# orting/image-feature-extraction

Hardware: AMD Instinct MI355X
Metric: Mvoxels/sec Hessian+eig, 512^3 fp32 3-scale (higher is better)
Workload: dtype f32 storage / f64 line recurrences

## Files before the change

### image-feature-extraction_amd/csrc/ife_capi.hip

```cpp
#include "../../include/ife_hip.h"

#include <hip/hip_runtime.h>

#include <algorithm>
#include <cmath>
#include <cstdarg>
#include <cstdio>
#include <cstdlib>
#include <cstring>
#include <map>
#include <new>
#include <string>
#include <tuple>
#include <type_traits>
#include <vector>

#include "feature_kernels.hpp"
#include "iir_types.hpp"
#include "stats_kernels.hpp"
#include "distance_kernels.hpp"
#include "dense_kernels.hpp"
#define IFE_IIR_NS iir_exact
#define IFE_IIR_FMA 0
#include "iir_kernels.inc"
// ... 359 lines not shown
DerivCoef deriv_coeffs(const ife_volume_desc *v, int dscale_mode) {
  DerivCoef d;
  const double sp[3] = {v->sx, v->sy, v->sz};
  for (int a = 0; a < 3; ++a) {
    const double s1 = 1.0 / sp[a];
    const double s2 = dscale_mode == 1 ? s1 * s1 : s1;
    d.m1[a] = -0.5 * s1;
    d.p1[a] = 0.5 * s1;
    d.a2[a] = 1.0 * s2;
    d.b2[a] = -2.0 * s2;
    d.c2[a] = 1.0 * s2;
  }
  return d;
}

IirGeom geom_for_axis(const ife_volume_desc *v, int axis) {
  IirGeom g;
  g.in_w = 0; g.in_group = 0; g.in_nz = 0;
  const int64_t nx = v->nx, ny = v->ny, nz = v->nz;
  if (axis == 2) {
    g.n = nz; g.nlines = nx * ny; g.sstride = nx * ny; g.inner = nx * ny; g.outer = 0;
  } else if (axis == 1) {
    g.n = ny; g.nlines = nx * nz; g.sstride = nx; g.inner = nx; g.outer = nx * ny;
  } else {
    g.n = nx; g.nlines = ny * nz; g.sstride = 1; g.inner = 1; g.outer = nx;
  }
  return g;
}

size_t ck_pairs(int64_t n, int K) { return (size_t)((n + K - 1) / K); }

int ensure_ck(ife_ctx *ctx, const ife_volume_desc *v, int njobs) {
  const int K = 8;
  size_t need_y = 0;
  for (int a = 0; a < 3; ++a) {
    IirGeom g = geom_for_axis(v, a);
    const size_t np = ck_pairs(g.n, K);
    need_y = std::max(need_y, np * 4 * (size_t)g.nlines * sizeof(double));
  }
  for (int j = 0; j < njobs; ++j) {
    int rc = ensure(ctx, ctx->ck_y[j], need_y);
    if (rc) return rc;
  }
  return IFE_OK;
}

int ensure_slots(ife_ctx *ctx, const ife_volume_desc *v, int nslots) {
  const size_t nb = (size_t)(v->nx * v->ny * v->nz) * sizeof(float);
  for (int s = 0; s < nslots; ++s)
    for (int i = 0; i < 4; ++i) {
      int rc = ensure(ctx, ctx->fld[s][i], nb);
      if (rc) return rc;
    }
  return IFE_OK;
}

struct ZSweepSrc {
  const void *img, *msk;
  int img_dtype, msk_dtype;
  float *tc, *cf;
  int nf;
  bool write_src;
};
int launch_iir(ife_ctx *ctx, const ife_volume_desc *v, int axis, int njobs,
               const float *const *in, float *const *out, const double *sigma,
               int in_y_chunks = 1, const int *order = nullptr ,
               const float *const *in2 = nullptr, const ZSweepSrc *zs = nullptr) {
  if (njobs < 1 || njobs > IIR_MAX_JOBS) return fail(ctx, IFE_E_ARG, "bad job count %d", njobs);
  IirGeom g = geom_for_axis(v, axis);
  if (in_y_chunks > 1) {
    if (axis != 0) return fail(ctx, IFE_E_ARG, "Y-chunked input is only read by the x pass");
    if (v->ny % in_y_chunks || (v->ny / in_y_chunks) % 64)
      return fail(ctx, IFE_E_SIZE, "Y-chunked input needs ny/chunks to be a multiple of 64");
    g.in_w = in_y_chunks;
    g.in_group = v->ny / in_y_chunks;
    g.in_nz = v->nz;
  }
  if ((int64_t)2 * 16 * g.sstride * 4 >= (int64_t)1 << 31 ||
      g.outer * 4 >= (int64_t)1 << 32 || g.nlines * 8 * 3 >= (int64_t)1 << 32)
    return fail(ctx, IFE_E_SIZE, "volume too large for the 32-bit offsets of the line kernels");
  if (in2 && (axis == 0 || 2 * njobs > IIR_MAX_JOBS || ctx->iir_ckpt != 2))
    return fail(ctx, IFE_E_ARG, "the paired form runs on the strided axes with at most %d jobs", IIR_MAX_JOBS / 2);
  if (zs && (axis != 2 || in2 || order || ctx->iir_ckpt != 2 || zs->nf < 1 || zs->nf > 2 || njobs % zs->nf ||
             njobs / zs->nf > IFE_MAX_SLOTS || !zs->img || !zs->tc || (zs->nf == 2 && (!zs->msk || !zs->cf))))
    return fail(ctx, IFE_E_ARG, "the shared sweep runs the Z pass of up to %d scales with pair checkpoints", IFE_MAX_SLOTS);
  int rc = ensure_ck(ctx, v, in2 ? 2 * njobs : njobs);
  if (rc) return rc;
  if (zs && (rc = ensure(ctx, ctx->zs_rec, (size_t)zs->nf * (size_t)g.nlines * sizeof(uint32_t)))) return rc;
  uint32_t any_const = 0;
  const double sp = axis == 0 ? v->sx : axis == 1 ? v->sy : v->sz;
  IirJobs jobs;
  memset(&jobs, 0, sizeof jobs);
  for (int j = 0; j < njobs; ++j) {
    if (!in[j] || !out[j] || in[j] == out[j]) return fail(ctx, IFE_E_ARG, "bad job buffers");
    if ((reinterpret_cast<uintptr_t>(in[j]) | reinterpret_cast<uintptr_t>(out[j])) % 4)
      return fail(ctx, IFE_E_ARG, "field pointers must be aligned to 4 bytes");
    jobs.j[j].in = in[j];
    jobs.j[j].out = out[j];
    jobs.j[j].ck_y = (double *)ctx->ck_y[j].p;
    if (in2) {
      if (!in2[j] || in2[j] == out[j] || reinterpret_cast<uintptr_t>(in2[j]) % 4)
        return fail(ctx, IFE_E_ARG, "bad denominator buffer");
      jobs.j[j].in2 = in2[j];
      jobs.j[j].ck_y2 = (double *)ctx->ck_y[njobs + j].p;
    }
    if (gauss_coeffs_order(sigma[j], sp, order ? order[j] : 0, &jobs.j[j].c))
      return fail(ctx, IFE_E_ARG, "spacing is suspiciously small");
    jobs.j[j].const_lines = 0;
    if (ctx->const_lines && !ctx->iir_fma && (!order || order[j] == 0)) {
      const int64_t len = axis == 0 ? v->nx : axis == 1 ? v->ny : v->nz;
      const std::tuple<double, double, int64_t> key(sigma[j], sp, len);
      auto it = ctx->const_flags.find(key);
      if (it == ctx->const_flags.end()) {
        if (ctx->const_flags.size() > 256) ctx->const_flags.clear();
        it = ctx->const_flags.emplace(key, const_line_flags(jobs.j[j].c, len)).first;
      }
      jobs.j[j].const_lines = it->second;
    }
    any_const |= jobs.j[j].const_lines;
    if (zs) jobs.j[j].line_rec = (const uint32_t *)ctx->zs_rec.p + (size_t)(j % zs->nf) * (size_t)g.nlines;
  }
  g.njobs = njobs;
  g.ngroups = (int32_t)((g.nlines + (in2 ? 127 : 255)) / (in2 ? 128 : 256));
  const dim3 grid((unsigned)((g.ngroups + 7) / 8 * 8 * njobs), 1, 1);
  const int sblock = ctx->iir_block ? ctx->iir_block : 12;
  if (zs) {
    ProfScope pz(ctx, KK_PREP);
    ZSweepArgs za;
    za.img = zs->img; za.msk = zs->msk; za.tc = zs->tc; za.cf = zs->cf;
    za.rec = (uint32_t *)ctx->zs_rec.p;
    za.nf = zs->nf; za.write_src = zs->write_src ? 1 : 0; za.track = any_const ? 1 : 0;
    IirGeom gs = g;
    gs.njobs = zs->nf;
    const dim3 sgrid((unsigned)((gs.ngroups + 7) / 8 * 8 * zs->nf), 1, 1);
    with_iir_kernels(ctx->iir_fma, [&](auto ks) {
      using KS = decltype(ks);
      with_const<8, 10, 12, 16>(sblock, [&](auto K) {
        with_const<1, 2, 3>(njobs / zs->nf, [&](auto S) {
          auto launch = [&](auto ti, auto tm) {
            hipLaunchKernelGGL((KS::template sweep_z<decltype(K)::value, decltype(S)::value, decltype(ti), decltype(tm)>),
                               sgrid, dim3(256), 0, ctx->stream, jobs, gs, za);
          };
          auto with_mask = [&](auto ti) {
            if (zs->msk && zs->msk_dtype == IFE_U16) launch(ti, uint16_t{});
            else launch(ti, uint8_t{});
          };
          if (zs->img_dtype == IFE_F32) with_mask(float{});
          else with_mask(int16_t{});
        });
      });
    });
    IFE_HIP(ctx, hipGetLastError());
  }
  ProfScope ps(ctx, axis == 2 ? KK_IIR_Z : axis == 1 ? KK_IIR_Y : KK_IIR_X);
  with_iir_kernels(ctx->iir_fma, [&](auto ks) {
    using KS = decltype(ks);
    auto launch = [&](auto kernel) { hipLaunchKernelGGL(kernel, grid, dim3(256), 0, ctx->stream, jobs, g); };
    if (zs)
      with_const<8, 10, 12, 16>(sblock, [&](auto K) { launch(KS::template strided<decltype(K)::value, false, true>); });
    else if (in2)
      with_const<8, 10, 12, 16>(sblock, [&](auto K) { launch(KS::template strided<decltype(K)::value, true, false>); });
    else if (axis == 0)
      with_const<8, 16>(ctx->iir_block, [&](auto K) { launch(KS::template contig<decltype(K)::value>); });
    else if (ctx->iir_ckpt == 1)
      with_const<8, 16>(ctx->iir_block, [&](auto K) { launch(KS::template strided1<decltype(K)::value>); });
    else
      with_const<8, 10, 12, 16>(sblock, [&](auto K) { launch(KS::template strided<decltype(K)::value, false, false>); });
// ... 1006 lines not shown
```

### image-feature-extraction_amd/csrc/iir_kernels.inc

```
#include <hip/hip_runtime.h>
#include <stdint.h>

#include <hip/hip_runtime.h>
#include <stdint.h>

#include <stddef.h>

#include <type_traits>

#include "iir_types.hpp"

#if IFE_IIR_FMA
#define IFE_MADD(a, b, acc) fma((a), (b), (acc))
#else
#define IFE_MADD(a, b, acc) ((a) * (b) + (acc))
#endif

namespace ife {
namespace IFE_IIR_NS {




struct IirCoefMain {
// ... 29 lines not shown
  double y1, y2, y3, y4;
};

template <typename C>
__device__ __forceinline__ double causal_step(CausalState &s, double xin, const C &c) {
  const double a = IFE_MADD(s.x3, c.N3, IFE_MADD(s.x2, c.N2, IFE_MADD(s.x1, c.N1, xin * c.N0)));
  const double t = IFE_MADD(s.y4, c.D4, IFE_MADD(s.y3, c.D3, IFE_MADD(s.y2, c.D2, s.y1 * c.D1)));
  const double y = a - t;
  s.x3 = s.x2; s.x2 = s.x1; s.x1 = xin;
  s.y4 = s.y3; s.y3 = s.y2; s.y2 = s.y1; s.y1 = y;
  return y;
}
__device__ __forceinline__ double causal_step_edge(CausalState &s, double xin, const IirCoef &c,
                                                   int64_t i) {
  const double d1 = i < 1 ? c.BN1 : c.D1;
  const double d2 = i < 2 ? c.BN2 : c.D2;
  const double d3 = i < 3 ? c.BN3 : c.D3;
  const double d4 = i < 4 ? c.BN4 : c.D4;
  const double a = IFE_MADD(s.x3, c.N3, IFE_MADD(s.x2, c.N2, IFE_MADD(s.x1, c.N1, xin * c.N0)));
  const double t = IFE_MADD(s.y4, d4, IFE_MADD(s.y3, d3, IFE_MADD(s.y2, d2, s.y1 * d1)));
  const double y = a - t;
  s.x3 = s.x2; s.x2 = s.x1; s.x1 = xin;
  s.y4 = s.y3; s.y3 = s.y2; s.y2 = s.y1; s.y1 = y;
  return y;
}
template <typename C>
__device__ __forceinline__ double anti_step(AntiState &s, double xin, const C &c) {
  const double a = IFE_MADD(s.x4, c.M4, IFE_MADD(s.x3, c.M3, IFE_MADD(s.x2, c.M2, s.x1 * c.M1)));
  const double t = IFE_MADD(s.y4, c.D4, IFE_MADD(s.y3, c.D3, IFE_MADD(s.y2, c.D2, s.y1 * c.D1)));
  const double y = a - t;
  s.x4 = s.x3; s.x3 = s.x2; s.x2 = s.x1; s.x1 = xin;
  s.y4 = s.y3; s.y3 = s.y2; s.y2 = s.y1; s.y1 = y;
  return y;
}
__device__ __forceinline__ double anti_step_edge(AntiState &s, double xin, const IirCoef &c,
                                                 int64_t i, int64_t n) {
  const double d1 = i + 1 >= n ? c.BM1 : c.D1;
  const double d2 = i + 2 >= n ? c.BM2 : c.D2;
  const double d3 = i + 3 >= n ? c.BM3 : c.D3;
  const double d4 = i + 4 >= n ? c.BM4 : c.D4;
  const double a = IFE_MADD(s.x4, c.M4, IFE_MADD(s.x3, c.M3, IFE_MADD(s.x2, c.M2, s.x1 * c.M1)));
  const double t = IFE_MADD(s.y4, d4, IFE_MADD(s.y3, d3, IFE_MADD(s.y2, d2, s.y1 * d1)));
  const double y = a - t;
  s.x4 = s.x3; s.x3 = s.x2; s.x2 = s.x1; s.x1 = xin;
  s.y4 = s.y3; s.y3 = s.y2; s.y2 = s.y1; s.y1 = y;
  return y;
}

using rsrc_t = __amdgpu_buffer_rsrc_t;

__device__ __forceinline__ int64_t uniform64(int64_t v) {
  const uint32_t lo = __builtin_amdgcn_readfirstlane((uint32_t)(uint64_t)v);
  const uint32_t hi = __builtin_amdgcn_readfirstlane((uint32_t)((uint64_t)v >> 32));
  return (int64_t)(((uint64_t)hi << 32) | lo);
}
__device__ __forceinline__ rsrc_t make_rsrc(const void *ubase) {
  return __builtin_amdgcn_make_buffer_rsrc(const_cast<void *>(ubase), 0, -1, 0x00020000);
}
__device__ __forceinline__ rsrc_t make_rsrc_null(const void *ubase) {
  return __builtin_amdgcn_make_buffer_rsrc(const_cast<void *>(ubase), 0, 0, 0x00020000);
}
__device__ __forceinline__ rsrc_t make_rsrc_range(const void *ubase, uint32_t range) {
  return __builtin_amdgcn_make_buffer_rsrc(const_cast<void *>(ubase), 0, (int)range, 0x00020000);
}
__device__ __forceinline__ uint32_t mask_lt(int a, int b) {
  uint32_t m;
  asm("s_sub_i32 %0, %1, %2\n\ts_ashr_i32 %0, %0, 31" : "=s"(m) : "s"(a), "s"(b) : "scc");
  return m;
}
#if defined(IFE_DIAG_NO_OUT)
#define IFE_OUT_RSRC make_rsrc_null
#define IFE_OUT_RSRC_RANGE(ptr, range) make_rsrc_null(ptr)
#else
#define IFE_OUT_RSRC make_rsrc
#define IFE_OUT_RSRC_RANGE(ptr, range) make_rsrc_range((ptr), (range))
#endif
#if defined(IFE_DIAG_NO_CK)
#define IFE_CK_RSRC make_rsrc_null
#else
#define IFE_CK_RSRC make_rsrc
#endif
#if defined(IFE_DIAG_NO_IN)
#define IFE_IN_RSRC make_rsrc_null
#else
#define IFE_IN_RSRC make_rsrc
#endif
__device__ __forceinline__ float buf_ld_f32(rsrc_t r, uint32_t voff, uint32_t soff) {
  return __builtin_bit_cast(float, __builtin_amdgcn_raw_buffer_load_b32(r, voff, soff, 0));
}
#ifndef IFE_IN2_AUX
#define IFE_IN2_AUX 0
#endif
__device__ __forceinline__ float buf_ld_last_f32(rsrc_t r, uint32_t voff, uint32_t soff) {
  return __builtin_bit_cast(float, __builtin_amdgcn_raw_buffer_load_b32(r, voff, soff, IFE_IN2_AUX));
}
__device__ __forceinline__ void buf_st_f32(rsrc_t r, uint32_t voff, uint32_t soff, float v) {
  __builtin_amdgcn_raw_buffer_store_b32(__builtin_bit_cast(uint32_t, v), r, voff, soff, 0);
}
#ifndef IFE_OUT_AUX
#define IFE_OUT_AUX 2
#endif
__device__ __forceinline__ void buf_st_out_f32(rsrc_t r, uint32_t voff, uint32_t soff, float v) {
  __builtin_amdgcn_raw_buffer_store_b32(__builtin_bit_cast(uint32_t, v), r, voff, soff, IFE_OUT_AUX);
}
typedef uint32_t u32x2 __attribute__((ext_vector_type(2)));
typedef uint32_t u32x4 __attribute__((ext_vector_type(4)));
#ifndef IFE_CK_ST_AUX
#define IFE_CK_ST_AUX 0
#endif
#ifndef IFE_CK_LD_AUX
#define IFE_CK_LD_AUX 0
#endif
__device__ __forceinline__ double ck_ld_f64(rsrc_t r, uint32_t voff, uint32_t soff) {
  return __builtin_bit_cast(double, __builtin_amdgcn_raw_buffer_load_b64(r, voff, soff, IFE_CK_LD_AUX));
}
__device__ __forceinline__ void ck_st_f64(rsrc_t r, uint32_t voff, uint32_t soff, double v) {
  __builtin_amdgcn_raw_buffer_store_b64(__builtin_bit_cast(u32x2, v), r, voff, soff, IFE_CK_ST_AUX);
}
__device__ __forceinline__ float ck_ld_f32(rsrc_t r, uint32_t voff, uint32_t soff) {
  return __builtin_bit_cast(float, __builtin_amdgcn_raw_buffer_load_b32(r, voff, soff, IFE_CK_LD_AUX));
}
__device__ __forceinline__ void ck_st_f32(rsrc_t r, uint32_t voff, uint32_t soff, float v) {
  __builtin_amdgcn_raw_buffer_store_b32(__builtin_bit_cast(uint32_t, v), r, voff, soff, IFE_CK_ST_AUX);
}
__device__ __forceinline__ double buf_ld_f64(rsrc_t r, uint32_t voff, uint32_t soff) {
  return __builtin_bit_cast(double, __builtin_amdgcn_raw_buffer_load_b64(r, voff, soff, 0));
}
__device__ __forceinline__ void buf_st_f64(rsrc_t r, uint32_t voff, uint32_t soff, double v) {
  __builtin_amdgcn_raw_buffer_store_b64(__builtin_bit_cast(u32x2, v), r, voff, soff, 0);
}
template <typename T>
__device__ __forceinline__ float buf_ld_as_f32(rsrc_t r, uint32_t voff, uint32_t soff);
template <>
__device__ __forceinline__ float buf_ld_as_f32<float>(rsrc_t r, uint32_t voff, uint32_t soff) {
  return buf_ld_f32(r, voff, soff);
}
template <>
__device__ __forceinline__ float buf_ld_as_f32<uint8_t>(rsrc_t r, uint32_t voff, uint32_t soff) {
  return (float)(uint8_t)__builtin_amdgcn_raw_buffer_load_b8(r, voff, soff, 0);
}
template <>
__device__ __forceinline__ float buf_ld_as_f32<uint16_t>(rsrc_t r, uint32_t voff, uint32_t soff) {
  return (float)(uint16_t)__builtin_amdgcn_raw_buffer_load_b16(r, voff, soff, 0);
}
template <>
__device__ __forceinline__ float buf_ld_as_f32<int16_t>(rsrc_t r, uint32_t voff, uint32_t soff) {
  return (float)(int16_t)__builtin_amdgcn_raw_buffer_load_b16(r, voff, soff, 0);
}

__device__ __forceinline__ bool const_line_response(uint32_t bits, uint32_t flags, float &resp) {
  resp = __builtin_bit_cast(float, bits);
  if (bits == 0u) return (flags & 1u) != 0;
  if (bits == 0x3f800000u) return (flags & 2u) != 0;
  if (bits == 0x80000000u) {
    if (flags & 8u) resp = 0.0f;
    return (flags & 12u) != 0;
  }
  return false;
}
__device__ __forceinline__ bool same_bits(float a, float b) {
  return __builtin_bit_cast(uint32_t, a) == __builtin_bit_cast(uint32_t, b);
}


struct SrcF32 {
  const float *p;
  struct At { rsrc_t a; };
  __device__ __forceinline__ At at(int64_t u) const { return At{IFE_IN_RSRC(p + u)}; }
// ... 469 lines not shown
      }
      if (b > 0) {
#pragma unroll
        for (int j = 0; j < K; ++j) causal_step(s, (double)xb[j], c);
      } else {
        const double x0 = (double)xb[0];
        s.x1 = s.x2 = s.x3 = x0;
        s.y1 = s.y2 = s.y3 = s.y4 = x0;
#pragma unroll
        for (int j = 0; j < K; ++j) causal_step_edge(s, (double)xb[j], c, j);
      }
      if (live) ck_store(ck, b + 1, nl, Lw, lane, s);
#pragma unroll
      for (int j = 0; j < K; ++j) xb[j] = xn[j];
    }
  }

  {
    float xa[K], na[K];
    float h1 = 0.f, h2 = 0.f, h3 = 0.f, nh1 = 0.f, nh2 = 0.f, nh3 = 0.f;
    AntiState a;
    CausalState sc, sn;
    sc.y1 = sc.y2 = sc.y3 = sc.y4 = 0.0;
    sn = sc;
    auto load_hist = [&](int64_t b, float &q1, float &q2, float &q3) {
      const auto B = src.at(wbase + (b * K - 3) * st);
      q3 = src.ld(B, voff, 0u);
      q2 = src.ld(B, voff, sst);
      q1 = src.ld(B, voff, 2u * sst);
    };
    {
      const int64_t i0 = (nb - 1) * K;
      const auto B = src.at(wbase + i0 * st);
      const uint32_t lastj = (uint32_t)(n - 1 - i0);
#pragma unroll
      for (int j = 0; j < K; ++j)
        xa[j] = src.ld(B, voff, ((uint32_t)j < lastj ? (uint32_t)j : lastj) * sst);
      if (nb > 1) {
        load_hist(nb - 1, h1, h2, h3);
        ck_load(ck, nb - 1, nl, Lw, live ? lane : 0u, sc);
      }
      const double xN = (double)xa[K - 1];
      a.x1 = a.x2 = a.x3 = a.x4 = xN;
      a.y1 = a.y2 = a.y3 = a.y4 = xN;
    }
    for (int64_t b = nb - 1; b >= 0; --b) {
      const int64_t i0 = b * K;
      if (b > 0) {
        const auto B = src.at(wbase + (i0 - K) * st);
#pragma unroll
        for (int j = 0; j < K; ++j) na[j] = src.ld(B, voff, (uint32_t)j * sst);
        if (b > 1) {
          load_hist(b - 1, nh1, nh2, nh3);
          ck_load(ck, b - 1, nl, Lw, live ? lane : 0u, sn);
        }
      }
      CausalState s;
      if (b > 0) {
        s.y1 = sc.y1; s.y2 = sc.y2; s.y3 = sc.y3; s.y4 = sc.y4;
        s.x1 = (double)h1; s.x2 = (double)h2; s.x3 = (double)h3;
      } else {
        const double x0 = (double)xa[0];
        s.x1 = s.x2 = s.x3 = x0;
        s.y1 = s.y2 = s.y3 = s.y4 = x0;
      }
      const bool edge = (b == 0) || (i0 + K + 4 > n);
      double cz[K];
      causal_run<K, true>(s, xa, cz, c, i0, n, edge);
      anti_run<K>(a, xa, cz, c, i0, n, edge);
      if (live) {
        const rsrc_t ro = IFE_OUT_RSRC(out + wbase + i0 * st);
#pragma unroll
        for (int j = 0; j < K; ++j)
          if (!edge || i0 + j < n) buf_st_out_f32(ro, voff * 4u, (uint32_t)j * sst * 4u, xa[j]);
      }
#pragma unroll
      for (int j = 0; j < K; ++j) xa[j] = na[j];
      h1 = nh1; h2 = nh2; h3 = nh3;
      sc.y1 = sn.y1; sc.y2 = sn.y2; sc.y3 = sn.y3; sc.y4 = sn.y4;
    }
  }
}

template <typename T>
__device__ __forceinline__ uint32_t buf_ld_raw(rsrc_t r, uint32_t voff, uint32_t soff);
template <>
__device__ __forceinline__ uint32_t buf_ld_raw<float>(rsrc_t r, uint32_t voff, uint32_t soff) {
  return __builtin_amdgcn_raw_buffer_load_b32(r, voff, soff, 0);
}
template <>
__device__ __forceinline__ uint32_t buf_ld_raw<int16_t>(rsrc_t r, uint32_t voff, uint32_t soff) {
  return (uint32_t)(uint16_t)__builtin_amdgcn_raw_buffer_load_b16(r, voff, soff, 0);
}
template <>
__device__ __forceinline__ uint32_t buf_ld_raw<uint16_t>(rsrc_t r, uint32_t voff, uint32_t soff) {
  return (uint32_t)(uint16_t)__builtin_amdgcn_raw_buffer_load_b16(r, voff, soff, 0);
}
template <>
__device__ __forceinline__ uint32_t buf_ld_raw<uint8_t>(rsrc_t r, uint32_t voff, uint32_t soff) {
  return (uint32_t)(uint8_t)__builtin_amdgcn_raw_buffer_load_b8(r, voff, soff, 0);
}
template <typename T>
__device__ __forceinline__ float raw_as_f32(uint32_t r) {
  if constexpr (std::is_same<T, float>::value) return __builtin_bit_cast(float, r);
  else if constexpr (std::is_same<T, int16_t>::value) return (float)(int16_t)(uint16_t)r;
  else return (float)r;
}
struct SweepY {
  double y1, y2, y3, y4;
};
template <typename C>
__device__ __forceinline__ void sweep_step(SweepY &s, double x1, double x2, double x3, double xin, const C &c) {
  const double a = IFE_MADD(x3, c.N3, IFE_MADD(x2, c.N2, IFE_MADD(x1, c.N1, xin * c.N0)));
  const double t = IFE_MADD(s.y4, c.D4, IFE_MADD(s.y3, c.D3, IFE_MADD(s.y2, c.D2, s.y1 * c.D1)));
  const double y = a - t;
  s.y4 = s.y3; s.y3 = s.y2; s.y2 = s.y1; s.y1 = y;
}
struct SweepCoef {
  double N0, N1, N2, N3, D1, D2, D3, D4;
};
template <int K, int NS, typename TI, typename TM>
__global__ __launch_bounds__(256, K <= 12 ? 4 : 3) void iir_sweep_z_kernel(IirJobs jobs, IirGeom g, ZSweepArgs a) {
  const IirBlock blk = iir_block_of(g, blockIdx.x);
  if (!blk.live) return;
  const uint32_t lane = threadIdx.x & 63u;
  const int64_t Lw = uniform64((int64_t)blk.group * blockDim.x + (int64_t)(threadIdx.x & ~63u));
  if (Lw >= g.nlines) return;
  const uint32_t f = blk.job, nf = (uint32_t)a.nf;
  const bool is_den = f != 0u;
  const bool has_mask = a.msk != nullptr;
  const int64_t n = g.n, nl = g.nlines;
  int64_t L = Lw + lane;
  if (L >= nl) L = nl - 1;
  const uint32_t cl = (uint32_t)(L - Lw);
  const uint32_t sst = (uint32_t)nl;
  const int nb = (int)((n + K - 1) / K);
  const int np = (nb + 1) / 2;
  const int nfp = np - 1;
  float *const dst = reinterpret_cast<float *>(uniform64(reinterpret_cast<int64_t>(is_den ? a.cf : a.tc)));
  const uint32_t rd_img = is_den ? 0u : 0xffffffffu;
  const uint32_t rd_msk = has_mask ? 0xffffffffu : 0u;
  const uint32_t wr_src = a.write_src != 0 ? 0xffffffffu : 0u;

  SweepCoef c[NS];
  double *cky[NS];
#pragma unroll
  for (int k = 0; k < NS; ++k) {
    const IirJob &J = jobs.j[(uint32_t)k * nf + f];
    c[k] = SweepCoef{J.c.N0, J.c.N1, J.c.N2, J.c.N3, J.c.D1, J.c.D2, J.c.D3, J.c.D4};
    cky[k] = J.ck_y;
  }

  uint32_t ri[K], rm[K];
  float v[K];
  SweepY s[NS];
  double x1 = 0.0, x2 = 0.0, x3 = 0.0;
  bool cst = true;
  uint32_t ref = 0u;

  constexpr int G = K % 4 == 0 ? 4 : 2;
  const int ni = (int)n;
  const uint32_t nlu = (uint32_t)nl, lwu = (uint32_t)Lw;
  auto range_of = [&](int row, uint32_t esize) -> uint32_t {
    int rows = ni - row;
    rows = rows < 0 ? 0 : rows;
    rows = rows > 2 * K ? 2 * K : rows;
    const uint32_t one = rows > 0 ? 1u : 0u;
    return ((uint32_t)rows * nlu - one * lwu) * esize;
  };
  auto load_blk = [&](int b, uint32_t (&ri)[K], uint32_t (&rm)[K]) {
    __builtin_amdgcn_sched_barrier(0);
#pragma unroll
    for (int q = 0; q < K; q += G) {
      const int row = b * K + q;
      const int64_t e0 = Lw + (int64_t)row * nl;
      const rsrc_t dI = make_rsrc_range(static_cast<const TI *>(a.img) + e0, range_of(row, sizeof(TI)) & rd_img);
#pragma unroll
      for (int j = 0; j < G; ++j)
        ri[q + j] = buf_ld_raw<TI>(dI, cl * (uint32_t)sizeof(TI), (uint32_t)j * sst * (uint32_t)sizeof(TI));
    }
#pragma unroll
    for (int q = 0; q < K; q += G) {
      const int row = b * K + q;
      const int64_t e0 = Lw + (int64_t)row * nl;
      const rsrc_t dM = make_rsrc_range(static_cast<const TM *>(has_mask ? a.msk : a.img) + e0,
                                        range_of(row, sizeof(TM)) & rd_msk);
#pragma unroll
      for (int j = 0; j < G; ++j)
        rm[q + j] = buf_ld_raw<TM>(dM, cl * (uint32_t)sizeof(TM), (uint32_t)j * sst * (uint32_t)sizeof(TM));
    }
  };
  auto take_blk = [&](int b, const uint32_t (&ri)[K], const uint32_t (&rm)[K]) {
    __builtin_amdgcn_sched_barrier(0);
    if (is_den) {
#pragma unroll
      for (int j = 0; j < K; ++j) v[j] = raw_as_f32<TM>(rm[j]);
    } else if (has_mask) {
#pragma unroll
      for (int j = 0; j < K; ++j) v[j] = raw_as_f32<TI>(ri[j]) * raw_as_f32<TM>(rm[j]);
    } else {
#pragma unroll
      for (int j = 0; j < K; ++j) v[j] = raw_as_f32<TI>(ri[j]);
    }
#pragma unroll
    for (int q = 0; q < K; q += G) {
      const int row = b * K + q;
      const rsrc_t dO = make_rsrc_range(dst + Lw + (int64_t)row * nl, range_of(row, 4u) & wr_src);
#pragma unroll
      for (int j = 0; j < G; ++j) buf_st_f32(dO, cl * 4u, (uint32_t)j * sst * 4u, v[q + j]);
    }
  };
  auto track = [&]() {
    if (a.track) {
#pragma unroll
      for (int j = 0; j < K; ++j) cst = cst && __builtin_bit_cast(uint32_t, v[j]) == ref;
    }
  };
  auto run = [&](int j0, int j1) {
#pragma unroll
    for (int j = j0; j < j1; ++j) {
      const double xin = (double)v[j];
#pragma unroll
      for (int k = 0; k < NS; ++k) sweep_step(s[k], x1, x2, x3, xin, c[k]);
      x3 = x2; x2 = x1; x1 = xin;
    }
  };
  auto store_state = [&](int slot) {
#pragma unroll
    for (int k = 0; k < NS; ++k) {
      double *const base = reinterpret_cast<double *>(uniform64(reinterpret_cast<int64_t>(cky[k])));
      const rsrc_t ry = IFE_CK_RSRC(base + ((int64_t)slot * 4) * nl + Lw);
      const uint32_t sy = (uint32_t)nl * 8u;
      ck_st_f64(ry, cl * 8u, 0u, s[k].y1);
      ck_st_f64(ry, cl * 8u, sy, s[k].y2);
      ck_st_f64(ry, cl * 8u, 2u * sy, s[k].y3);
      ck_st_f64(ry, cl * 8u, 3u * sy, s[k].y4);
    }
  };

  load_blk(0, ri, rm);
  if (nfp > 0) {
    take_blk(0, ri, rm);
    load_blk(1, ri, rm);
    ref = __builtin_bit_cast(uint32_t, v[0]);
    {
      const double e0 = (double)v[0];
#pragma unroll
      for (int k = 0; k < NS; ++k) {
        const IirCoef ce = edge_coefs((uint32_t)k * nf + f);
        CausalState e;
        e.x1 = e.x2 = e.x3 = e0;
        e.y1 = e.y2 = e.y3 = e.y4 = e0;
#pragma unroll
        for (int j = 0; j < K; ++j) causal_step_edge(e, (double)v[j], ce, j);
        s[k] = SweepY{e.y1, e.y2, e.y3, e.y4};
      }
      x1 = (double)v[K - 1]; x2 = (double)v[K - 2]; x3 = (double)v[K - 3];
    }
    track();
    take_blk(1, ri, rm);
    load_blk(2, ri, rm);
    run(0, K);
    track();
    for (int p = 1; p < nfp; ++p) {
      take_blk(2 * p, ri, rm);
      load_blk(2 * p + 1, ri, rm);
      run(0, 3);
      store_state(p);
      run(3, K);
      track();
      take_blk(2 * p + 1, ri, rm);
      load_blk(2 * p + 2, ri, rm);
      run(0, K);
      track();
    }
    store_state(np - 1);
    if (a.track) a.rec[(int64_t)f * nl + L] = cst ? ref : ZSWEEP_NOT_CONST;
  }
  take_blk(2 * nfp, ri, rm);
  load_blk(2 * nfp + 1, ri, rm);
  take_blk(2 * nfp + 1, ri, rm);
}

template <int W>
struct XTile {
  static constexpr int PITCH = W + 4;
  static constexpr int FLOATS = 64 * PITCH;
};

__device__ __forceinline__ void wave_lds_sync() {
  asm volatile("s_waitcnt lgkmcnt(0)" ::: "memory");
  __builtin_amdgcn_wave_barrier();
}

template <int W, int AUX = 0>
__device__ __forceinline__ void xtile_fill(const float *rows, float *tile, uint32_t lane,
                                           int64_t nrows, int64_t pitch, int64_t i0, int64_t n,
                                           bool vec_ok) {
  constexpr int P = XTile<W>::PITCH;
  constexpr int V = W / 4;
  constexpr int LPI = 64 / V;
  if (vec_ok && i0 + W <= n) {
    const rsrc_t r4 = make_rsrc(rows + i0);
    u32x4 v[V];
#pragma unroll
    for (int r = 0; r < V; ++r) {
      uint32_t row = (lane / V) + r * LPI;
      if ((int64_t)row >= nrows) row = (uint32_t)(nrows - 1);
      const uint32_t off = (row * (uint32_t)pitch + 4u * (lane % V)) * 4u;
      v[r] = __builtin_amdgcn_raw_buffer_load_b128(r4, off, 0u, AUX);
    }
#pragma unroll
    for (int r = 0; r < V; ++r)
      *reinterpret_cast<u32x4 *>(tile + ((lane / V) + r * LPI) * P + 4 * (lane % V)) = v[r];
  } else {
#pragma clang loop unroll(disable)
    for (int e = 0; e < W; ++e) {
      const uint32_t idx = e * 64 + lane;
      uint32_t row = idx / W;
      const uint32_t col = idx % W;
      const uint32_t trow = row;
      if ((int64_t)row >= nrows) row = (uint32_t)(nrows - 1);
      int64_t i = i0 + col;
      if (i >= n) i = n - 1;
      tile[trow * P + col] = rows[(int64_t)row * pitch + i];
    }
  }
  wave_lds_sync();
}

template <int W, int K>
__device__ __forceinline__ void xtile_get(const float *tile, uint32_t lane, int h, float (&xb)[K]) {
  constexpr int P = XTile<W>::PITCH;
#pragma unroll
  for (int q = 0; q < K / 4; ++q) {
    const float4 t = *reinterpret_cast<const float4 *>(tile + lane * P + h * K + 4 * q);
    xb[4 * q + 0] = t.x; xb[4 * q + 1] = t.y; xb[4 * q + 2] = t.z; xb[4 * q + 3] = t.w;
  }
}
template <int W, int K>
__device__ __forceinline__ void xtile_put(float *tile, uint32_t lane, int h, const float (&xb)[K]) {
  constexpr int P = XTile<W>::PITCH;
#pragma unroll
  for (int q = 0; q < K / 4; ++q)
    *reinterpret_cast<float4 *>(tile + lane * P + h * K + 4 * q) =
        make_float4(xb[4 * q + 0], xb[4 * q + 1], xb[4 * q + 2], xb[4 * q + 3]);
}

template <int W>
__device__ __forceinline__ void xtile_drain(float *rows, float *tile, uint32_t lane,
                                            int64_t nrows, int64_t pitch, int64_t i0, int64_t n,
                                            bool vec_ok) {
  constexpr int P = XTile<W>::PITCH;
  constexpr int V = W / 4;
  constexpr int LPI = 64 / V;
  wave_lds_sync();
  if (vec_ok && i0 + W <= n) {
    const rsrc_t r4 = make_rsrc(rows + i0);
#pragma unroll
    for (int r = 0; r < V; ++r) {
      const uint32_t row = (lane / V) + r * LPI;
      const u32x4 v = *reinterpret_cast<const u32x4 *>(tile + row * P + 4 * (lane % V));
      const uint32_t off = (row * (uint32_t)pitch + 4u * (lane % V)) * 4u;
      if ((int64_t)row < nrows) __builtin_amdgcn_raw_buffer_store_b128(v, r4, off, 0u, IFE_OUT_AUX);
// ... 706 lines not shown
```

Before: 47320.

## Specialize Z sweep kernel per field type and stream block pointers incrementally

Splits the shared Z-sweep kernel into compile-time variants for numerator, denominator and plain fields, so unused image or mask loads are dropped entirely instead of being masked by a zero range. Buffer base pointers and checkpoint pointers now advance incrementally, and coefficients are read straight from the kernarg segment. It also adds configurable prefetch depth for the image, mask and denominator streams (default 1), a cheaper OR-based constant tracker, and a scalar-asm range computation. The costs are larger code size from three instantiations and tighter argument validation in the host check.

After: 47590 (median of 6 runs). Within noise of the previous version (+0.6%).

```diff
diff --git a/image-feature-extraction_amd/csrc/ife_capi.hip b/image-feature-extraction_amd/csrc/ife_capi.hip
--- a/image-feature-extraction_amd/csrc/ife_capi.hip
+++ b/image-feature-extraction_amd/csrc/ife_capi.hip
@@ -465,7 +465,8 @@
   if (in2 && (axis == 0 || 2 * njobs > IIR_MAX_JOBS || ctx->iir_ckpt != 2))
     return fail(ctx, IFE_E_ARG, "the paired form runs on the strided axes with at most %d jobs", IIR_MAX_JOBS / 2);
   if (zs && (axis != 2 || in2 || order || ctx->iir_ckpt != 2 || zs->nf < 1 || zs->nf > 2 || njobs % zs->nf ||
-             njobs / zs->nf > IFE_MAX_SLOTS || !zs->img || !zs->tc || (zs->nf == 2 && (!zs->msk || !zs->cf))))
+             njobs / zs->nf > IFE_MAX_SLOTS || !zs->img || !zs->tc || (zs->nf == 2) != (zs->msk != nullptr) ||
+             (zs->nf == 2 && !zs->cf)))
     return fail(ctx, IFE_E_ARG, "the shared sweep runs the Z pass of up to %d scales with pair checkpoints", IFE_MAX_SLOTS);
   int rc = ensure_ck(ctx, v, in2 ? 2 * njobs : njobs);
   if (rc) return rc;
diff --git a/image-feature-extraction_amd/csrc/iir_kernels.inc b/image-feature-extraction_amd/csrc/iir_kernels.inc
--- a/image-feature-extraction_amd/csrc/iir_kernels.inc
+++ b/image-feature-extraction_amd/csrc/iir_kernels.inc
@@ -135,8 +135,10 @@
 #endif
 #if defined(IFE_DIAG_NO_IN)
 #define IFE_IN_RSRC make_rsrc_null
+#define IFE_IN_RSRC_RANGE(ptr, range) make_rsrc_null(ptr)
 #else
 #define IFE_IN_RSRC make_rsrc
+#define IFE_IN_RSRC_RANGE(ptr, range) make_rsrc_range((ptr), (range))
 #endif
 __device__ __forceinline__ float buf_ld_f32(rsrc_t r, uint32_t voff, uint32_t soff) {
   return __builtin_bit_cast(float, __builtin_amdgcn_raw_buffer_load_b32(r, voff, soff, 0));
@@ -772,6 +774,24 @@
   }
 }
 
+#ifndef IFE_ZS_DEPTH_IMG
+#define IFE_ZS_DEPTH_IMG 1
+#endif
+#ifndef IFE_ZS_DEPTH_MSK
+#define IFE_ZS_DEPTH_MSK 1
+#endif
+#ifndef IFE_ZS_DEPTH_DEN
+#define IFE_ZS_DEPTH_DEN 1
+#endif
+#ifndef IFE_ZS_WAVES
+#define IFE_ZS_WAVES 4
+#endif
+#ifndef IFE_ZS_SRC_AUX
+#define IFE_ZS_SRC_AUX 0
+#endif
+__device__ __forceinline__ void buf_st_src_f32(rsrc_t r, uint32_t voff, uint32_t soff, float v) {
+  __builtin_amdgcn_raw_buffer_store_b32(__builtin_bit_cast(uint32_t, v), r, voff, soff, IFE_ZS_SRC_AUX);
+}
 template <typename T>
 __device__ __forceinline__ uint32_t buf_ld_raw(rsrc_t r, uint32_t voff, uint32_t soff);
 template <>
@@ -809,16 +829,27 @@
 struct SweepCoef {
   double N0, N1, N2, N3, D1, D2, D3, D4;
 };
-template <int K, int NS, typename TI, typename TM>
-__global__ __launch_bounds__(256, K <= 12 ? 4 : 3) void iir_sweep_z_kernel(IirJobs jobs, IirGeom g, ZSweepArgs a) {
-  const IirBlock blk = iir_block_of(g, blockIdx.x);
-  if (!blk.live) return;
+__device__ __forceinline__ SweepCoef sweep_coefs(uint32_t job, double *&ck_y) {
+  typedef __attribute__((address_space(4))) const char kchar;
+  kchar *ka = (kchar *)__builtin_amdgcn_kernarg_segment_ptr() + (size_t)job * sizeof(IirJob);
+  asm volatile("" : "+s"(ka));
+  typedef __attribute__((address_space(4))) const double kdouble;
+  typedef double *dptr;
+  typedef __attribute__((address_space(4))) const dptr kdptr;
+  ck_y = *(kdptr *)(ka + offsetof(IirJob, ck_y));
+  kdouble *d = (kdouble *)(ka + offsetof(IirJob, c));
+  return SweepCoef{d[0], d[1], d[2], d[3], d[4], d[5], d[6], d[7]};
+}
+constexpr int ZS_NUM = 0;
+constexpr int ZS_DEN = 1;
+constexpr int ZS_PLAIN = 2;
+template <int K, int NS, typename TI, typename TM, int F>
+__device__ __forceinline__ void sweep_z_body(const IirJobs &jobs, const IirGeom &g, const ZSweepArgs &a,
+                                             const int64_t Lw) {
+  constexpr bool RD_IMG = F != ZS_DEN, RD_MSK = F != ZS_PLAIN;
+  constexpr uint32_t NF = F == ZS_PLAIN ? 1u : 2u, FI = F == ZS_DEN ? 1u : 0u;
+  constexpr int DI = IFE_ZS_DEPTH_IMG, DM = F == ZS_DEN ? IFE_ZS_DEPTH_DEN : IFE_ZS_DEPTH_MSK;
   const uint32_t lane = threadIdx.x & 63u;
-  const int64_t Lw = uniform64((int64_t)blk.group * blockDim.x + (int64_t)(threadIdx.x & ~63u));
-  if (Lw >= g.nlines) return;
-  const uint32_t f = blk.job, nf = (uint32_t)a.nf;
-  const bool is_den = f != 0u;
-  const bool has_mask = a.msk != nullptr;
   const int64_t n = g.n, nl = g.nlines;
   int64_t L = Lw + lane;
   if (L >= nl) L = nl - 1;
@@ -827,83 +858,91 @@
   const int nb = (int)((n + K - 1) / K);
   const int np = (nb + 1) / 2;
   const int nfp = np - 1;
-  float *const dst = reinterpret_cast<float *>(uniform64(reinterpret_cast<int64_t>(is_den ? a.cf : a.tc)));
-  const uint32_t rd_img = is_den ? 0u : 0xffffffffu;
-  const uint32_t rd_msk = has_mask ? 0xffffffffu : 0u;
+  float *const dst = reinterpret_cast<float *>(uniform64(reinterpret_cast<int64_t>(F == ZS_DEN ? a.cf : a.tc)));
   const uint32_t wr_src = a.write_src != 0 ? 0xffffffffu : 0u;
 
   SweepCoef c[NS];
   double *cky[NS];
 #pragma unroll
   for (int k = 0; k < NS; ++k) {
-    const IirJob &J = jobs.j[(uint32_t)k * nf + f];
-    c[k] = SweepCoef{J.c.N0, J.c.N1, J.c.N2, J.c.N3, J.c.D1, J.c.D2, J.c.D3, J.c.D4};
-    cky[k] = J.ck_y;
-  }
-
-  uint32_t ri[K], rm[K];
+    c[k] = sweep_coefs((uint32_t)k * NF + FI, cky[k]);
+  }
+
+  uint32_t ri[RD_IMG ? DI : 1][K], rm[RD_MSK ? DM : 1][K];
   float v[K];
   SweepY s[NS];
   double x1 = 0.0, x2 = 0.0, x3 = 0.0;
-  bool cst = true;
   uint32_t ref = 0u;
 
   constexpr int G = K % 4 == 0 ? 4 : 2;
   const int ni = (int)n;
   const uint32_t nlu = (uint32_t)nl, lwu = (uint32_t)Lw;
-  auto range_of = [&](int row, uint32_t esize) -> uint32_t {
-    int rows = ni - row;
-    rows = rows < 0 ? 0 : rows;
-    rows = rows > 2 * K ? 2 * K : rows;
-    const uint32_t one = rows > 0 ? 1u : 0u;
-    return ((uint32_t)rows * nlu - one * lwu) * esize;
+  auto range_of = [&](int left, uint32_t esize) -> uint32_t {
+    uint32_t rows, one;
+    asm("s_max_i32 %0, %2, 0\n\ts_min_i32 %0, %0, %3\n\ts_min_i32 %1, %0, 1"
+        : "=&s"(rows), "=s"(one) : "s"(left), "i"(2 * K) : "scc");
+    return (rows * nlu - one * lwu) * esize;
   };
-  auto load_blk = [&](int b, uint32_t (&ri)[K], uint32_t (&rm)[K]) {
+  uint64_t pi = reinterpret_cast<uint64_t>(a.img) + (uint64_t)Lw * sizeof(TI);
+  uint64_t pm = reinterpret_cast<uint64_t>(a.msk) + (uint64_t)Lw * sizeof(TM);
+  uint64_t po = reinterpret_cast<uint64_t>(dst) + (uint64_t)Lw * 4u;
+  int rem = ni;
+  auto load_img = [&](int left, uint32_t (&r)[K]) {
+    if constexpr (RD_IMG) {
+      __builtin_amdgcn_sched_barrier(0);
+#pragma unroll
+      for (int q = 0; q < K; q += G) {
+        const rsrc_t dI = IFE_IN_RSRC_RANGE(reinterpret_cast<const void *>(pi), range_of(left - q, sizeof(TI)));
+        pi += (uint64_t)((uint32_t)G * nlu * (uint32_t)sizeof(TI));
+#pragma unroll
+        for (int j = 0; j < G; ++j)
+          r[q + j] = buf_ld_raw<TI>(dI, cl * (uint32_t)sizeof(TI), (uint32_t)j * sst * (uint32_t)sizeof(TI));
+      }
+    }
+  };
+  auto load_msk = [&](int left, uint32_t (&r)[K]) {
+    if constexpr (RD_MSK) {
+      __builtin_amdgcn_sched_barrier(0);
+#pragma unroll
+      for (int q = 0; q < K; q += G) {
+        const rsrc_t dM = IFE_IN_RSRC_RANGE(reinterpret_cast<const void *>(pm), range_of(left - q, sizeof(TM)));
+        pm += (uint64_t)((uint32_t)G * nlu * (uint32_t)sizeof(TM));
+#pragma unroll
+        for (int j = 0; j < G; ++j)
+          r[q + j] = buf_ld_raw<TM>(dM, cl * (uint32_t)sizeof(TM), (uint32_t)j * sst * (uint32_t)sizeof(TM));
+      }
+    }
+  };
+  auto take_blk = [&](const uint32_t (&qi)[K], const uint32_t (&qm)[K]) {
     __builtin_amdgcn_sched_barrier(0);
 #pragma unroll
+    for (int j = 0; j < K; ++j) {
+      if constexpr (F == ZS_DEN) v[j] = raw_as_f32<TM>(qm[j]);
+      else if constexpr (F == ZS_NUM) v[j] = raw_as_f32<TI>(qi[j]) * raw_as_f32<TM>(qm[j]);
+      else v[j] = raw_as_f32<TI>(qi[j]);
+    }
+#pragma unroll
     for (int q = 0; q < K; q += G) {
-      const int row = b * K + q;
-      const int64_t e0 = Lw + (int64_t)row * nl;
-      const rsrc_t dI = make_rsrc_range(static_cast<const TI *>(a.img) + e0, range_of(row, sizeof(TI)) & rd_img);
-#pragma unroll
-      for (int j = 0; j < G; ++j)
-        ri[q + j] = buf_ld_raw<TI>(dI, cl * (uint32_t)sizeof(TI), (uint32_t)j * sst * (uint32_t)sizeof(TI));
-    }
-#pragma unroll
-    for (int q = 0; q < K; q += G) {
-      const int row = b * K + q;
-      const int64_t e0 = Lw + (int64_t)row * nl;
-      const rsrc_t dM = make_rsrc_range(static_cast<const TM *>(has_mask ? a.msk : a.img) + e0,
-                                        range_of(row, sizeof(TM)) & rd_msk);
-#pragma unroll
-      for (int j = 0; j < G; ++j)
-        rm[q + j] = buf_ld_raw<TM>(dM, cl * (uint32_t)sizeof(TM), (uint32_t)j * sst * (uint32_t)sizeof(TM));
-    }
+      const rsrc_t dO = IFE_OUT_RSRC_RANGE(reinterpret_cast<void *>(po), range_of(rem - q, 4u) & wr_src);
+      po += (uint64_t)((uint32_t)G * nlu * 4u);
+#pragma unroll
+      for (int j = 0; j < G; ++j) buf_st_src_f32(dO, cl * 4u, (uint32_t)j * sst * 4u, v[q + j]);
+    }
+    rem -= K;
   };
-  auto take_blk = [&](int b, const uint32_t (&ri)[K], const uint32_t (&rm)[K]) {
-    __builtin_amdgcn_sched_barrier(0);
-    if (is_den) {
-#pragma unroll
-      for (int j = 0; j < K; ++j) v[j] = raw_as_f32<TM>(rm[j]);
-    } else if (has_mask) {
-#pragma unroll
-      for (int j = 0; j < K; ++j) v[j] = raw_as_f32<TI>(ri[j]) * raw_as_f32<TM>(rm[j]);
-    } else {
-#pragma unroll
-      for (int j = 0; j < K; ++j) v[j] = raw_as_f32<TI>(ri[j]);
-    }
-#pragma unroll
-    for (int q = 0; q < K; q += G) {
-      const int row = b * K + q;
-      const rsrc_t dO = make_rsrc_range(dst + Lw + (int64_t)row * nl, range_of(row, 4u) & wr_src);
-#pragma unroll
-      for (int j = 0; j < G; ++j) buf_st_f32(dO, cl * 4u, (uint32_t)j * sst * 4u, v[q + j]);
-    }
+  auto next_blk = [&](auto par) {
+    constexpr int P = decltype(par)::value;
+    take_blk(ri[RD_IMG ? P % DI : 0], rm[RD_MSK ? P % DM : 0]);
+    load_img(rem - (DI - 1) * K, ri[RD_IMG ? P % DI : 0]);
+    load_msk(rem - (DM - 1) * K, rm[RD_MSK ? P % DM : 0]);
   };
+  const std::integral_constant<int, 0> even;
+  const std::integral_constant<int, 1> odd;
+  uint32_t dif = 0u;
   auto track = [&]() {
     if (a.track) {
 #pragma unroll
-      for (int j = 0; j < K; ++j) cst = cst && __builtin_bit_cast(uint32_t, v[j]) == ref;
+      for (int j = 0; j < K; ++j) dif |= __builtin_bit_cast(uint32_t, v[j]) ^ ref;
     }
   };
   auto run = [&](int j0, int j1) {
@@ -915,11 +954,15 @@
       x3 = x2; x2 = x1; x1 = xin;
     }
   };
-  auto store_state = [&](int slot) {
+  uint64_t pc[NS];
+#pragma unroll
+  for (int k = 0; k < NS; ++k)
+    pc[k] = (uint64_t)uniform64(reinterpret_cast<int64_t>(cky[k])) + ((uint64_t)nlu * 4u + (uint64_t)Lw) * 8u;
+  auto store_state = [&]() {
 #pragma unroll
     for (int k = 0; k < NS; ++k) {
-      double *const base = reinterpret_cast<double *>(uniform64(reinterpret_cast<int64_t>(cky[k])));
-      const rsrc_t ry = IFE_CK_RSRC(base + ((int64_t)slot * 4) * nl + Lw);
+      const rsrc_t ry = IFE_CK_RSRC(reinterpret_cast<void *>(pc[k]));
+      pc[k] += (uint64_t)(nlu * 32u);
       const uint32_t sy = (uint32_t)nl * 8u;
       ck_st_f64(ry, cl * 8u, 0u, s[k].y1);
       ck_st_f64(ry, cl * 8u, sy, s[k].y2);
@@ -928,16 +971,18 @@
     }
   };
 
-  load_blk(0, ri, rm);
+#pragma unroll
+  for (int d = 0; d < DI; ++d) load_img(ni - d * K, ri[RD_IMG ? d : 0]);
+#pragma unroll
+  for (int d = 0; d < DM; ++d) load_msk(ni - d * K, rm[RD_MSK ? d : 0]);
   if (nfp > 0) {
-    take_blk(0, ri, rm);
-    load_blk(1, ri, rm);
+    next_blk(even);
     ref = __builtin_bit_cast(uint32_t, v[0]);
     {
       const double e0 = (double)v[0];
 #pragma unroll
       for (int k = 0; k < NS; ++k) {
-        const IirCoef ce = edge_coefs((uint32_t)k * nf + f);
+        const IirCoef ce = edge_coefs((uint32_t)k * NF + FI);
         CausalState e;
         e.x1 = e.x2 = e.x3 = e0;
         e.y1 = e.y2 = e.y3 = e.y4 = e0;
@@ -948,28 +993,35 @@
       x1 = (double)v[K - 1]; x2 = (double)v[K - 2]; x3 = (double)v[K - 3];
     }
     track();
-    take_blk(1, ri, rm);
-    load_blk(2, ri, rm);
+    next_blk(odd);
     run(0, K);
     track();
     for (int p = 1; p < nfp; ++p) {
-      take_blk(2 * p, ri, rm);
-      load_blk(2 * p + 1, ri, rm);
+      next_blk(even);
       run(0, 3);
-      store_state(p);
+      store_state();
       run(3, K);
       track();
-      take_blk(2 * p + 1, ri, rm);
-      load_blk(2 * p + 2, ri, rm);
+      next_blk(odd);
       run(0, K);
       track();
     }
-    store_state(np - 1);
-    if (a.track) a.rec[(int64_t)f * nl + L] = cst ? ref : ZSWEEP_NOT_CONST;
-  }
-  take_blk(2 * nfp, ri, rm);
-  load_blk(2 * nfp + 1, ri, rm);
-  take_blk(2 * nfp + 1, ri, rm);
+    store_state();
+    if (a.track) a.rec[(int64_t)FI * nl + L] = dif == 0u ? ref : ZSWEEP_NOT_CONST;
+  }
+  next_blk(even);
+  next_blk(odd);
+}
+
+template <int K, int NS, typename TI, typename TM>
+__global__ __launch_bounds__(256, K <= 12 ? IFE_ZS_WAVES : 3) void iir_sweep_z_kernel(IirJobs jobs, IirGeom g, ZSweepArgs a) {
+  const IirBlock blk = iir_block_of(g, blockIdx.x);
+  if (!blk.live) return;
+  const int64_t Lw = uniform64((int64_t)blk.group * blockDim.x + (int64_t)(threadIdx.x & ~63u));
+  if (Lw >= g.nlines) return;
+  if (blk.job != 0u) sweep_z_body<K, NS, TI, TM, ZS_DEN>(jobs, g, a, Lw);
+  else if (a.msk != nullptr) sweep_z_body<K, NS, TI, TM, ZS_NUM>(jobs, g, a, Lw);
+  else sweep_z_body<K, NS, TI, TM, ZS_PLAIN>(jobs, g, a, Lw);
 }
 
 template <int W>
```
